# diku-kmc/kleenexlang

Hardware: AMD Instinct MI355X
Metric: input GB/s + % HBM-read roofline, apache_log.kex over 10 GiB synthetic log (higher is better)
Workload: dtype u8

## Files before the change

### kleenexlang_amd/csrc/engine/kx_dfkernels.inc

```

struct DfDev {
  const uint32_t* img; uint32_t words;
  uint32_t off_pool, deadh, esch, starth, K, C;
  const uint16_t* start_of_state;
  uint32_t orig_c4, hshift;
  uint32_t short_consts, debug;
  uint32_t nstates;
  uint32_t J;
  uint32_t wide;
  const uint4* sl_fmap;
  const uint32_t* sl_back; const uint8_t* sl_nleaves; const uint8_t* sl_fin_leaf; const uint8_t* sl_cls;
  const uint32_t* sl_pcoff; const uint8_t* sl_pcpool; const uint32_t* sl_pend; const uint32_t* sl_defoff; const uint32_t* sl_defpc; const uint16_t* sl_q;
  uint32_t sl_Lm, sl_npc, sl_on;
};
constexpr uint32_t DF_HOLE_MAX = 4096, DF_HOLE_FIRST = 1024, DF_SL_LEAVES = 32;
struct __attribute__((aligned(8))) DfRec { uint32_t x, y; };
constexpr uint32_t DFREC_OWN = 0x80000000u, DFREC_HOLE = 0x80000000u, DFREC_HOLE_FIRST = 0x40000000u;
constexpr uint32_t DF_MERGE_WINDOW_MAX = 64;
constexpr uint32_t DF_STEP_MAX = 126, DF_HOLE_LEN_MAX = 0xFFFFu, DF_HOLE_CNT_MAX = 0x3FFFu, DF_WBASE_PIECES = 32;
constexpr DfRec dfrec_pack(uint32_t start, uint32_t middle, uint32_t lenA, uint32_t len, uint32_t kA, uint32_t kB) {
  return DfRec{(start >> 3) | ((middle >> 3) << 13) | (kA << 26), len | (lenA << 13) | (kB << 25)};
}
constexpr DfRec dfrec_pack_hole(uint32_t side_first, uint32_t entries, bool first, uint32_t len) {
  return DfRec{side_first, len | (entries << 16) | (first ? DFREC_HOLE_FIRST : 0u) | DFREC_HOLE};
// ... 457 lines not shown
    for (uint32_t t = 0; t < plen; ++t) {
      if (t == HALF) { mid = h; lenA = len; kA = kc; }
      const uint2 e = L.ent(h + L.c8(in[pos + t]));
      const uint32_t nh = e.x & 0xFFFFu;
      if (nh == dead) { atomicMin(&flags->fail_pos, (unsigned long long)(pos + t)); return; }
      if (nh == esc) { flags->df_esc = 1; return; }
      h = nh; len += e.y >> 24; kc += (e.y >> 23) & 1u;
    }
    if (plen <= HALF) { mid = h; lenA = len; kA = kc; }
    if (kc > 0) atomicMax(&flags->emit_kmax, kc);
    if (((pos >> 6) & (DF_WBASE_PIECES - 1)) == 0) wbase[(pos >> 6) / DF_WBASE_PIECES] = cum;
    rec[pos >> 6] = dfrec_pack(h0, mid, lenA, len, kA, kc - kA);
    cum += len; pos += plen;
  }
  spill[m] = cum;
  if (head_len == n) flags->end_state = h;
}

__global__ void k_dlen(uint32_t nblk, const uint32_t* __restrict__ own, const uint32_t* __restrict__ spill, uint32_t* __restrict__ len,
                       unsigned long long* __restrict__ wsum) {
  __shared__ unsigned long long red[1024];
  const uint32_t m = blockIdx.x * blockDim.x + threadIdx.x;
  uint32_t mylen = 0;
  if (m < nblk) { mylen = own[m] + spill[m]; len[m] = mylen; }
  red[threadIdx.x] = mylen;
  __syncthreads();
  for (uint32_t s = blockDim.x >> 1; s > 0; s >>= 1) {
    if (threadIdx.x < s) red[threadIdx.x] += red[threadIdx.x + s];
    __syncthreads();
  }
  if (threadIdx.x == 0) wsum[blockIdx.x] = red[0];
}

template <bool GENERAL>
__global__ void k_dmap(const uint8_t* __restrict__ in, uint64_t n, uint32_t q_in, uint64_t cap, uint8_t* __restrict__ map_out,
                       uint32_t* __restrict__ status, DevTables T) {
  extern __shared__ __attribute__((aligned(16))) uint32_t smem[];
  Lds L = stage_tables<GENERAL>(T, smem);
  if (blockIdx.x || threadIdx.x) return;
  __shared__ uint8_t M[2][256];
  const uint32_t C = T.nclasses;
  uint32_t h = (OFF_FWD + q_in * C * 4) >> T.hshift, cur = 0;
  uint32_t nl = T.nleaves[q_in];
  for (uint32_t l = 0; l < nl; ++l) M[0][l] = (uint8_t)l;
  uint64_t pos = 0;
  bool constant = nl == 1, dead = false;
  while (pos < n && pos < cap && !constant && !dead) {
    const uint64_t a8 = pos & ~7ull;
    uint64_t x = 0;
    if (a8 + 8 <= n) { const uint2 v = *reinterpret_cast<const uint2*>(in + a8); x = (uint64_t)v.x | ((uint64_t)v.y << 32); }
    else for (uint64_t i = a8; i < n; ++i) x |= (uint64_t)in[i] << (8 * (i - a8));
    for (uint32_t b = (uint32_t)pos & 7u; b < 8u && pos < n && pos < cap && !constant; ++b, ++pos) {
      const uint32_t e = L.next(h, (uint32_t)(x >> (8 * b)) & 0xFFu);
      const uint32_t nh = e & 0xFFFFu;
      if (nh == T.deadh) { dead = true; break; }
      const uint32_t row = L.ra(e >> 16);
      const uint32_t nq = ((nh << T.hshift) - OFF_FWD) / (C * 4);
      const uint32_t nnl = T.nleaves[nq];
      constant = true;
      for (uint32_t l = 0; l < nnl; ++l) {
        const uint32_t p = (L.w(row + l * 4) >> 2) & 0xFFu;
        M[cur ^ 1][l] = M[cur][p < nl ? p : 0];
        constant = constant && M[cur ^ 1][l] == M[cur ^ 1][0];
      }
      cur ^= 1; h = nh; nl = nnl;
    }
// ... 26 lines not shown
  asm volatile("s_mov_b64 %[sv], exec\n"
               "v_cmpx_lt_u32_e32 vcc, 0, %[m]\n"
               "ds_write_b32 %[d], %[w0]\n"
               "v_cmpx_lt_u32_e32 vcc, 1, %[m]\n"
               "ds_write_b32 %[d], %[w1] offset:4\n"
               "v_cmpx_lt_u32_e32 vcc, 2, %[m]\n"
               "ds_write_b32 %[d], %[w2] offset:8\n"
               "v_cmpx_lt_u32_e32 vcc, 3, %[m]\n"
               "ds_write_b32 %[d], %[w3] offset:12\n"
               "s_mov_b64 exec, %[sv]\n"
               : [sv] "=&s"(sv) : [m] "v"(m), [d] "v"(d), [w0] "v"(w[0]), [w1] "v"(w[1]), [w2] "v"(w[2]), [w3] "v"(w[3]) : "vcc", "memory");
}

#ifndef KX_PRIO_CONSTANTS
#define KX_PRIO_CONSTANTS 2
#endif
#ifndef KX_PRIO_FLUSH
#define KX_PRIO_FLUSH 1
#endif
constexpr int HALF_BYTES = HALF;

template <int CONSTS>
__device__ __forceinline__ void df_step_gen(uint32_t& h, uint32_t byte_now, uint32_t byte_out, uint64_t& o, uint8_t* __restrict__ dst,
                                            const DfLds& L, const DfDev& D) {
  const uint2 e = L.ent(h + L.c8(byte_now));
  h = e.x & 0xFFFFu;
  const uint32_t cp = E_COPY(e.y), dl = e.y >> 24;
  if (cp) dst[o] = (uint8_t)byte_out;
  if (dl > cp) { const uint32_t src = D.off_pool + (E_AID(e.y) << 4); for (uint32_t i = 0; i < dl - cp; ++i) dst[o + cp + i] = L.base[src + i]; }
  o += dl;
}

template <int WAVES, int K, bool HALF = false>
__global__ __launch_bounds__(WAVES * 64) void k_demit(const uint8_t* __restrict__ in, uint64_t n, uint64_t blk, uint64_t blk_inv,
                                                      uint64_t npieces_total, const DfRec* __restrict__ rec, const uint32_t* __restrict__ wbase,
                                                      const uint32_t* __restrict__ spill, const unsigned long long* __restrict__ off,
                                                      Flags* __restrict__ flags, uint32_t stgb, uint32_t jbytes, uint32_t maxcnt,
                                                      uint8_t* __restrict__ out, const uint32_t* __restrict__ side, DfDev D) {
  extern __shared__ __attribute__((aligned(16))) uint32_t smem[];
  DfLds L = df_stage(D, smem);
  if ((uint32_t)(uintptr_t)smem != 0u) __builtin_trap();
  constexpr int NB = HALF ? HALF_BYTES : PIECE, NW = NB / 4;
  const uint32_t wave = threadIdx.x >> 6, lane = threadIdx.x & 63;
  const uint32_t stga = ((D.words + 3) & ~3u) * 4 + wave * (stgb + 16 + jbytes);
  uint8_t* stg = (uint8_t*)smem + stga;
  const uint32_t jarea = stga + stgb + 16;
  const uint64_t nunits = HALF ? npieces_total * 2 : npieces_total;
  const uint64_t nwi = (nunits + 63) / 64;
  const uint64_t oend_all = flags->total_len;
  const uint64_t one_piece_blocks = (uint64_t)__builtin_amdgcn_readfirstlane(blk == (uint64_t)PIECE ? 1 : 0);
  struct Operands { uint32_t w[NW]; uint32_t wp; uint2 r; uint32_t wb; uint64_t off0; uint32_t sp0; };
  auto request = [&](uint64_t it_, Operands& o) {
    if (it_ >= nwi) return;
    {
      const uint64_t itu = ((uint64_t)(uint32_t)__builtin_amdgcn_readfirstlane((int)(uint32_t)(it_ >> 32)) << 32) | (uint32_t)__builtin_amdgcn_readfirstlane((int)(uint32_t)it_);
      const uint64_t pf = itu * (HALF ? 32u : 64u);
      const uint64_t mf = __umul64hi(pf, blk_inv) + pf * one_piece_blocks;
      uint32_t vw, vm;
      asm("v_mov_b32 %0, %1" : "=v"(vw) : "s"((uint32_t)(pf / DF_WBASE_PIECES)));
      asm("v_mov_b32 %0, %1" : "=v"(vm) : "s"((uint32_t)mf));
      o.wb = wbase[vw]; o.off0 = off[vm]; o.sp0 = spill[vm];
    }
    const uint64_t u = it_ * 64 + lane;
    const bool ok = u < nunits;
    const uint64_t pc = HALF ? u >> 1 : u;
    const uint64_t ustart = ok ? (HALF ? pc * PIECE + (u & 1) * HALF_BYTES : pc * PIECE) : n;
    if constexpr (HALF) {
      if (ustart + HALF_BYTES <= n) {
        const uint4* p = reinterpret_cast<const uint4*>(in + ustart);
        const uint4 v0 = p[0], v1 = p[1];
        o.w[0] = v0.x; o.w[1] = v0.y; o.w[2] = v0.z; o.w[3] = v0.w; o.w[4] = v1.x; o.w[5] = v1.y; o.w[6] = v1.z; o.w[7] = v1.w;
      } else {
#pragma unroll
        for (int i = 0; i < NW; ++i) {
          uint32_t x = 0;
#pragma unroll
          for (int bb = 0; bb < 4; ++bb) { const uint64_t a = ustart + 4 * i + bb; if (a < n) x |= (uint32_t)in[a] << (8 * bb); }
          o.w[i] = x;
        }
      }
    } else load_piece(in, n, ustart, o.w);
    o.wp = *reinterpret_cast<const uint32_t*>(ok && ustart >= 4 ? in + ustart - 4 : reinterpret_cast<const uint8_t*>(D.img));
    o.r = *reinterpret_cast<const uint2*>(rec + (ok ? pc : 0));
  };
  Operands nx, cur;
  request((uint64_t)blockIdx.x * WAVES + wave, nx);
  cur = nx;
  unsigned long long tk[6] = {0, 0, 0, 0, 0, 0};
  auto stamp = [&]() -> unsigned long long {
    if (!(D.debug & 64u)) return 0ull;
    asm volatile("s_waitcnt vmcnt(0) lgkmcnt(0)" ::: "memory");
    return __builtin_amdgcn_s_memtime();
  };
  for (uint64_t it = (uint64_t)blockIdx.x * WAVES + wave; it < nwi; it += (uint64_t)gridDim.x * WAVES) {
    const unsigned long long t0 = stamp();
    const uint64_t unit = it * 64 + lane;
    const bool valid = unit < nunits;
    const uint64_t piece = HALF ? unit >> 1 : unit;
    const uint32_t half = HALF ? (uint32_t)unit & 1u : 0u;
    const uint64_t ustart = piece * PIECE + half * HALF_BYTES;
    const int plen = valid ? (int)(n <= ustart ? 0 : n - ustart < (uint64_t)NB ? n - ustart : NB) : 0;
    uint32_t w[NW];
#pragma unroll
    for (int i = 0; i < NW; ++i) w[i] = cur.w[i];
    const uint32_t wp = cur.wp;
    const DfRec rc{cur.r.x, cur.r.y};
    const bool hole = valid && dfrec_hole(rc);
    const uint32_t len = hole ? dfrec_hole_len(rc) : dfrec_len(rc), lenA = hole ? len : dfrec_lenA(rc);
    const uint32_t kA = HALF ? (half ? dfrec_kB(rc) : dfrec_kA(rc)) : dfrec_kA(rc), kB = HALF ? 0u : dfrec_kB(rc);
    const uint32_t hA = HALF ? (half ? dfrec_middle(rc) : dfrec_start(rc)) : dfrec_start(rc), hB = dfrec_middle(rc);
    const uint32_t ulen = valid ? (HALF ? (half ? len - lenA : lenA) : len) : 0u;
    const uint32_t before = wave_scan_incl(ulen) - ulen;
    const uint64_t obase = cur.off0 + (cur.wb & ~DFREC_OWN) + ((cur.wb & DFREC_OWN) ? cur.sp0 : 0u);
    const uint64_t ostart = valid ? obase + before : oend_all, oend = valid ? ostart + ulen : oend_all;
    const unsigned long long vmask = __ballot(valid);
    const uint32_t nvalid = (uint32_t)__popcll(vmask);
    uint32_t first = 0;
    bool taken = false;
    unsigned long long t2 = stamp();
    tk[0] += t2 - t0;
    if (hole && half == 0) {
      const uint32_t cntE = dfrec_hole_entries(rc), e0 = dfrec_hole_side(rc);
      uint64_t u = dfrec_hole_first(rc) ? piece * PIECE - K : piece * PIECE, o = ostart;
      for (uint32_t x = 0; x < cntE; ++x) {
        const uint32_t ee = side[e0 + x], pc = (ee >> 1) & 0x3FFFFFFFu;
        if (ee & 1u) out[o++] = in[u];
        if (pc < D.sl_npc) for (uint32_t b = D.sl_pcoff[pc]; b < D.sl_pcoff[pc + 1]; ++b) out[o++] = D.sl_pcpool[b];
        if (!(ee >> 31)) ++u;
      }
    }
    while (first < nvalid) {
      if (first == 0) request(it + (uint64_t)gridDim.x * WAVES, nx);
      const uint64_t gs = wave_read64(ostart, first);
      const uint64_t abase = gs & ~15ull;
      const bool fits = valid && lane >= first && (oend - abase) <= (uint64_t)stgb && plen == NB && !hole;
      const unsigned long long fm = __ballot(fits) >> first;
      uint32_t cnt = fm == ~0ull ? 64u - first : (uint32_t)__builtin_ctzll(~fm);
      if (cnt > maxcnt) cnt = maxcnt;
      if (cnt == 0) {
        if (lane == first && hole) {
        } else
        if (lane == first) {
          uint32_t h = hA;
          uint64_t o = ostart;
          for (int t = 0; t < plen; ++t) {
            const int ts = t - K;
            const uint32_t bn = (w[t >> 2] >> ((t & 3) * 8)) & 0xFFu;
            const uint32_t bo_ = ts >= 0 ? (w[ts >> 2] >> ((ts & 3) * 8)) & 0xFFu : (wp >> ((4 + ts) * 8)) & 0xFFu;
            df_step_gen<0>(h, bn, bo_, o, out, L, D);
          }
        }
        first += 1;
        continue;
      }
      const uint32_t lastl = first + cnt - 1;
      const bool active = lane >= first && lane <= lastl;
      const uint32_t o0 = stga + (uint32_t)(ostart - abase);
      const bool inplace = jbytes == 0;
      const uint32_t need = active ? (kA + kB) * 4u : 0u;
      const uint32_t incl = wave_scan_incl(need);
      const uint32_t jtotal = (uint32_t)__builtin_amdgcn_readlane((int)incl, 63);
      const bool jfit = !inplace && jtotal <= jbytes;
      const unsigned long long t3 = stamp();
      tk[2] += t3 - t2;
      if (active && jfit) {
        uint32_t oA = o0, pA = jarea + incl - need;
        if constexpr (HALF) {
          if (D.wide) { if constexpr (K == 1) piece_dfwalk1cw_k1(w, wp, hA, oA, pA); else piece_dfwalk1cw_k2(w, wp, hA, oA, pA); }
          else { if constexpr (K == 1) piece_dfwalk1c_k1(w, wp, hA, oA, pA); else piece_dfwalk1c_k2(w, wp, hA, oA, pA); }
        } else {
          uint32_t oB = o0 + lenA, pB = pA + 4u * kA;
          if (D.wide) {
            if constexpr (K == 1) piece_dfwalk2cw_k1(w, wp, hA, oA, hB, oB, pA, pB);
            else piece_dfwalk2cw_k2(w, wp, hA, oA, hB, oB, pA, pB);
          } else {
            if constexpr (K == 1) piece_dfwalk2c_k1(w, wp, hA, oA, hB, oB, pA, pB);
            else piece_dfwalk2c_k2(w, wp, hA, oA, hB, oB, pA, pB);
          }
        }
      }
      uint32_t njobs = jfit ? jtotal >> 2 : 0u;
      if (!jfit) {
        if (!inplace && lane == first) atomicAdd(&flags->emit_ovf, cnt);
        if (active) {
          for (int ch = 0; ch < (HALF ? 1 : 2); ++ch) {
            uint32_t h = ch ? hB : hA;
            uint64_t o = (uint64_t)(o0 - stga) + (ch ? lenA : 0u);
            for (int t = ch * HALF_BYTES; t < (ch + 1) * HALF_BYTES; ++t) {
              const int ts = t - K;
              const uint32_t bn = (w[t >> 2] >> ((t & 3) * 8)) & 0xFFu;
// ... 9 lines not shown
      __builtin_amdgcn_s_setprio(KX_PRIO_CONSTANTS);
      for (uint32_t j0 = 0; j0 < njobs; j0 += 64) {
        const uint32_t j = j0 + lane;
        uint32_t l = 0, d = 0, off0 = 0;
        if (j < njobs) {
          const uint32_t jw = *reinterpret_cast<const uint32_t*>((const uint8_t*)smem + jarea + 4 * j);
          const uint32_t e = *reinterpret_cast<const uint32_t*>(L.base + (jw & 0xFFFFu) + 4);
          const uint32_t cp = E_COPY(e);
          l = (e >> 24) - cp;
          d = stga + (((jw >> 16) - stga) & 0xFFFFu) + cp;
          off0 = D.off_pool + (E_AID(e) << 4);
        }
        const uint32_t tob = (0u - d) & 3u, nh = l < tob ? l : tob, rem = l - nh;
        const uint32_t src = off0 + nh * ((l + 15u) & ~15u), d1 = d + nh;
        const uint32_t v0 = *reinterpret_cast<const uint32_t*>(L.base + off0);
        uint4 wv = *reinterpret_cast<const uint4*>(L.base + src);
        put_bytes3(nh, d, v0);
        for (uint32_t base = 0;; base += 16) {
          const uint32_t left = rem > base ? rem - base : 0u, m = left >> 2 < 4u ? left >> 2 : 4u;
          const uint32_t w4[4] = {wv.x, wv.y, wv.z, wv.w};
          put_dwords4(m, d1 + base, w4);
          const uint32_t nt = left < 16u ? left & 3u : 0u;
          const uint32_t tw = m == 0 ? wv.x : m == 1 ? wv.y : m == 2 ? wv.z : wv.w;
          put_bytes3(nt, d1 + base + 4u * m, tw);
          if (!__any(rem > base + 16u)) break;
          wv = *reinterpret_cast<const uint4*>(L.base + src + base + 16u);
        }
      }
      wave_lds_fence();
      __builtin_amdgcn_s_setprio(KX_PRIO_FLUSH);
      const unsigned long long t5 = stamp();
      tk[4] += t5 - t4;
      if (lastl + 1 >= nvalid) { cur = nx; taken = true; }
      const uint64_t ge = wave_read64(oend, lastl);
      const uint64_t fs = (gs + 15) & ~15ull, fe = ge & ~15ull;
      if (fs >= fe) {
        for (uint64_t x = gs + lane; x < ge; x += 64) out[x] = stg[x - abase];
      } else {
        if (gs + lane < fs) out[gs + lane] = stg[gs + lane - abase];
        if (fe + lane < ge) out[fe + lane] = stg[fe + lane - abase];
        for (uint64_t x = fs + (uint64_t)lane * 16; x < fe; x += 1024)
          *reinterpret_cast<uint4*>(out + x) = *reinterpret_cast<const uint4*>(stg + (x - abase));
      }
      wave_lds_fence();
      __builtin_amdgcn_s_setprio(0);
      t2 = stamp();
      tk[5] += t2 - t5;
      first = lastl + 1;
    }
    if (!taken) cur = nx;
  }
  if ((D.debug & 64u) && lane == 0)
    for (int i = 0; i < 6; ++i) atomicAdd(&flags->dbg[i], tk[i]);
}
```

### kleenexlang_amd/csrc/engine/kx_engine.hip

```cpp
#include <hip/hip_runtime.h>
#include <fcntl.h>
#include <sys/stat.h>
#include <unistd.h>

#include <cerrno>
#include <condition_variable>
#include <cstdint>
#include <algorithm>
#include <deque>
#include <mutex>
#include <chrono>
#include <thread>
#include <cstdio>
#include <cstdlib>
#include <cstring>
#include <string>
#include <type_traits>
#include <vector>

#include "../../../include/kxhip.h"
#include "../../../include/kxp_format.h"
#include "kx_delayed.h"

namespace {
// ... 1798 lines not shown
    *out_len = olen;
    return 0;
  }
};

struct kx_program {
  std::vector<Stage> stages;
  void* actbuf[2][2] = {{nullptr, nullptr}, {nullptr, nullptr}};
  size_t actcap[2][2] = {{0, 0}, {0, 0}};
  kx_config cfg = [] { kx_config c{}; c.block_threads = 512; return c; }();
  std::vector<Arena*> arenas;
  void* stagebuf[2] = {nullptr, nullptr};
  size_t stagecap[2] = {0, 0};
  hipEvent_t ev[KX_NKERNELS + 1] = {};
  bool have_events = false;
  int ncu = 256;
  std::vector<ActionRunner*> act_runners;
  BatchWs* batch = nullptr;
  FieldWs* fields = nullptr;
  FieldListWs* field_list = nullptr;
};

struct kx_shard {
  kx_program* prog; Stage* st; uint32_t stage; Arena* arena = nullptr;
  const DevTables* T = nullptr;
  const uint8_t* in; uint64_t n; int is_first, is_last; hipStream_t stream;
  uint64_t seg; uint32_t nseg, nblk, Lc, ngroups;
  uint64_t* seg_pos; uint16_t* seg_state; uint16_t* chk; Flags* flags;
  uint8_t *bs_start, *bs_merged, *bs_mstart, *E, *d_map; uint32_t *bs_len, *len, *d_const, *ctot;
  PieceRec* prec; uint16_t* merge_piece;
  unsigned long long *off, *wsum, *woff;
  Flags hflags{}; uint64_t head_len = 0; bool have_end = false; uint64_t out_len = 0; uint32_t init_shift = 0, init_leaf = 0;
  uint32_t df_qin = 0;
  bool df = false; DfRec* dfrec = nullptr; uint32_t *df_wbase = nullptr, *df_own = nullptr, *df_spill = nullptr, *side = nullptr; uint32_t side_cap = 0; std::vector<uint8_t> df_tail; uint64_t df_body = 0;
  uint32_t endId() const {
    if (!df) return st->stateOf(hflags.end_state);
    const uint32_t i = st->df.indexOf(hflags.end_state);
    return i < st->df.states.size() ? st->df.states[i].q : st->q0;
  }
  kx_stats stats{};
};

namespace {

size_t pad4(size_t x) { return (x + 3) & ~(size_t)3; }

thread_local int g_force_jl = -1;

int parseStage(const uint8_t*& c, const uint8_t* end, Stage& S, const kx_config& cfg, bool dry = false) {
  if (end < c || (size_t)(end - c) < 64) return setErr(KX_E_BLOB, "truncated stage header");
  uint32_t h[16];
  memcpy(h, c, 64); c += 64;
  if (h[0] != KXP_STAGE_MAGIC) return setErr(KX_E_BLOB, "bad stage magic");
  const uint32_t nstates = h[1], C = h[2], q0 = h[3], nactions = h[5], nops = h[6], nconsts = h[7], cpl = h[8];
  const uint32_t Lm = h[9], nback = h[10], npc = h[11], pcpl = h[12], nsync = h[13];
  const size_t sc = (size_t)nstates * C;
  {
    const unsigned long long need = 256ull + pad4(sc * 2) + sc * 4 + (unsigned long long)nstates * 4 + ((unsigned long long)nactions + 1) * 4 +
                                    (unsigned long long)nops * 8 + ((unsigned long long)nconsts + 1) * 4 + pad4(cpl) + sc * 4 + 2 * pad4(nstates) +
                                    (unsigned long long)nback * Lm * 4 + ((unsigned long long)npc + 1) * 4 + pad4(pcpl) + (unsigned long long)Lm * 4 +
                                    (unsigned long long)nsync * C * 4 + (unsigned long long)nsync * 4;
    if (nstates > 0xFFFFu || C > 256 || Lm > 256 || need > (unsigned long long)(end - c)) return setErr(KX_E_BLOB, "truncated stage body");
  }
  const uint8_t* cls = c; c += 256;
  const uint16_t* delta = (const uint16_t*)c; c += pad4(sc * 2);
  c += sc * 4;
  c += (size_t)nstates * 4;
// ... 637 lines not shown

uint32_t kx_num_stages(const kx_program* p) { return p ? (uint32_t)p->stages.size() : 0; }
int kx_stage_has_actions(const kx_program* p, uint32_t stage) { return p && stage < p->stages.size() && p->stages[stage].act ? 1 : 0; }

static int shardBegin(kx_program* p, uint32_t stage, const void* d_in, size_t n, int is_first, int is_last,
                      void* stream, kx_shard** out, bool internal) {
  if (!p || !out || stage >= p->stages.size()) return setErr(KX_E_ARG, "bad program/stage");
  if (!internal && p->stages[stage].act) return setErr(KX_E_ARG, "a stage with register actions cannot be sharded (kx_stage_has_actions)");
  if (n && (!d_in || ((uintptr_t)d_in & 15))) return setErr(KX_E_ARG, "input must be 16-byte aligned");
  if ((uint64_t)n >> 38) return setErr(KX_E_ARG, "a shard holds at most 256 GiB (piece indices are 32-bit); stream larger inputs in windows");
  auto* s = new kx_shard;
  s->prog = p; s->st = &p->stages[stage]; s->stage = stage;
  s->T = s->st->has_alt && s->st->use_alt ? &s->st->Talt : &s->st->T;
  s->in = (const uint8_t*)d_in; s->n = n; s->is_first = is_first; s->is_last = is_last; s->stream = (hipStream_t)stream;
  s->seg = p->cfg.segment_bytes;
  if (s->seg == 0) {
    const uint64_t slots = (uint64_t)p->ncu * 1024;
    const uint64_t m = (n + slots * 65536 - 1) / (slots * 65536) ? (n + slots * 65536 - 1) / (slots * 65536) : 1;
    s->seg = ((n + m * slots - 1) / (m * slots) + 511) & ~(uint64_t)511;
    if (s->seg < 4096) s->seg = 4096;
  }
  uint64_t ns = n ? (n + s->seg - 1) / s->seg : 1;
  if (ns > 0x7FFFFFF0ull) { delete s; return setErr(KX_E_ARG, "input too large for the configured segment size"); }
  s->nseg = (uint32_t)ns; s->nblk = s->nseg; s->Lc = s->st->maxleaves;
  const uint32_t bt = p->cfg.block_threads;
  s->ngroups = (s->nblk + bt - 1) / bt;
  if (p->arenas.empty()) p->arenas.push_back(new Arena);
  s->arena = p->arenas.back(); p->arenas.pop_back();
  Arena& A = *s->arena;
  s->df = s->st->has_df && n > 0;
  if (s->df && s->st->df_given_up) s->df = false;
  if (s->df && s->st->df_skip) { s->df = false; --s->st->df_skip; }
  s->side_cap = s->df && s->st->D.sl_on ? (uint32_t)(n / 8 < (1u << 22) ? (n / 8 > (1u << 18) ? n / 8 : (1u << 18)) : (1u << 22)) : 0u;
  size_t need = 4096 + (s->df ? (n / PIECE + 16) * sizeof(DfRec) + (n / PIECE / DF_WBASE_PIECES + 8) * 4 + 256 + (size_t)s->nseg * 8 + 512 + (size_t)s->side_cap * 4 + 256 : 0) + (size_t)s->nseg * (8 + 2) + (n / HALF + 32) * 2 + sizeof(Flags) +
                (size_t)s->nblk * ((size_t)s->Lc * 5 + 3 + 4 + 8 + 2 + 4) + (size_t)s->ngroups * 16 + KX_MAX_LEAVES + 64 +
                (n / PIECE + 16) * 8 + 256 * 32;
  int rc = A.reserve(need);
  if (rc) { p->arenas.push_back(s->arena); delete s; return rc; }
  A.reset();
  s->seg_pos = A.take<uint64_t>(s->nseg); s->seg_state = A.take<uint16_t>(s->nseg);
  s->chk = A.take<uint16_t>(n / HALF + 32); s->flags = A.take<Flags>(1);
  s->bs_start = A.take<uint8_t>((size_t)s->nblk * s->Lc); s->bs_len = A.take<uint32_t>((size_t)s->nblk * s->Lc);
  s->bs_merged = A.take<uint8_t>(s->nblk); s->bs_mstart = A.take<uint8_t>(s->nblk); s->E = A.take<uint8_t>(s->nblk);
  s->len = A.take<uint32_t>(s->nblk); s->off = A.take<unsigned long long>(s->nblk);
  s->wsum = A.take<unsigned long long>(s->ngroups); s->woff = A.take<unsigned long long>(s->ngroups);
  s->d_map = A.take<uint8_t>(KX_MAX_LEAVES); s->d_const = A.take<uint32_t>(4);
  s->prec = A.take<PieceRec>(n / PIECE + 16);
  s->merge_piece = A.take<uint16_t>(s->nblk); s->ctot = A.take<uint32_t>(s->nblk);
  if (s->df) { s->dfrec = A.take<DfRec>(n / PIECE + 16); s->df_wbase = A.take<uint32_t>(n / PIECE / DF_WBASE_PIECES + 8); s->df_own = A.take<uint32_t>(s->nblk); s->df_spill = A.take<uint32_t>(s->nblk); s->side = s->side_cap ? A.take<uint32_t>(s->side_cap) : nullptr; }
  if (!p->have_events) {
    for (auto& e : p->ev) if (hipEventCreate(&e) != hipSuccess) { p->arenas.push_back(s->arena); delete s; return setErr(KX_E_HIP, "hipEventCreate failed"); }
    p->have_events = true;
  }
  s->stats.in_bytes = n;
  *out = s;
  return 0;
}

int kx_shard_begin(kx_program* p, uint32_t stage, const void* d_in, size_t n, int is_first, int is_last,
                   void* stream, kx_shard** out) {
  return shardBegin(p, stage, d_in, n, is_first, is_last, stream, out, false);
}

static int readFlags(kx_shard* s) {
  HIPCHECK(hipMemcpyAsync(&s->hflags, s->flags, sizeof(Flags), hipMemcpyDeviceToHost, s->stream));
  HIPCHECK(hipStreamSynchronize(s->stream));
  return 0;
}

static void fillFwd(kx_shard* s, kx_fwd_summary* out) {
  out->synced = s->have_end ? 1 : 0;
  out->end_state = s->have_end ? s->endId() : 0;
  out->head_len = s->head_len;
  out->fail_pos = s->hflags.fail_pos;
}

static int generalForward(kx_shard* s) {
  kx_program* p = s->prog; Stage& S = *s->st;
  const uint32_t bt = p->cfg.block_threads;
  const bool timing = p->cfg.collect_timing;
  const uint32_t grid = (s->nseg + bt - 1) / bt;
  if (timing) HIPCHECK(hipEventRecord(p->ev[1], s->stream));
// ... 224 lines not shown
#undef KX_LAUNCH_BACKLEN
  if (timing) HIPCHECK(hipEventRecord(p->ev[1], s->stream));
  HIPCHECK(hipGetLastError());
  if (!s->is_first) {
    hipLaunchKernelGGL(k_shard_map, dim3(1), dim3(64), 0, s->stream, s->nblk, nle, s->bs_start, s->bs_merged,
                       s->bs_mstart, s->Lc, s->d_map, s->d_const);
    HIPCHECK(hipMemcpyAsync(out->start_leaf, s->d_map, nle, hipMemcpyDeviceToHost, s->stream));
    HIPCHECK(hipMemcpyAsync(&out->constant, s->d_const, 4, hipMemcpyDeviceToHost, s->stream));
  }
  HIPCHECK(hipStreamSynchronize(s->stream));
  if (timing) s->stats.kernel_ms[KX_K_BACKLEN] = evMs(p->ev[0], p->ev[1]);
  return 0;
}

int kx_shard_resolve(kx_shard* s, uint32_t end_leaf, uint64_t* out_len) {
  if (!s || !out_len) return setErr(KX_E_ARG, "null argument");
  kx_program* p = s->prog; Stage& S = *s->st;
  if (s->is_last) end_leaf = S.h_fin_leaf[s->endId()];
  if (end_leaf >= S.h_nleaves[s->endId()]) return setErr(KX_E_ARG, "end leaf out of range");
  if (s->n == 0) {
    s->init_shift = s->is_first ? S.h_init_len[end_leaf] : 0;
    s->out_len = s->init_shift;
    *out_len = s->out_len;
    s->init_leaf = end_leaf;
    return 0;
  }
  const uint32_t bt = p->cfg.block_threads;
  const bool timing = p->cfg.collect_timing;
  if (s->df) {
    if (timing) HIPCHECK(hipEventRecord(p->ev[0], s->stream));
    hipLaunchKernelGGL(k_dlen, dim3(s->ngroups), dim3(bt), 0, s->stream, s->nblk, s->df_own, s->df_spill, s->len, s->wsum);
    hipLaunchKernelGGL(k_scan_groups, dim3(1), dim3(1024), 0, s->stream, s->ngroups, s->wsum, s->woff, s->flags);
    hipLaunchKernelGGL(k_scan_blocks, dim3(s->ngroups), dim3(bt), 0, s->stream, s->nblk, s->len, s->woff, s->off);
    if (timing) HIPCHECK(hipEventRecord(p->ev[1], s->stream));
    HIPCHECK(hipGetLastError());
    const uint32_t K = S.df.K;
    uint8_t lastb[kxdf::DF_MAX_K] = {0, 0, 0, 0};
    const uint32_t nb = s->n < K ? (uint32_t)s->n : K;
    HIPCHECK(hipMemcpyAsync(lastb + (K - nb), s->in + (s->n - nb), nb, hipMemcpyDeviceToHost, s->stream));
    int rc = readFlags(s);
    if (rc) return rc;
    if (timing) s->stats.kernel_ms[KX_K_RESOLVE] = evMs(p->ev[0], p->ev[1]);
    if (S.df.indexOf(s->hflags.end_state) >= S.df.states.size()) return setErr(KX_E_ARG, "internal: the shard did not end in a state of the delayed form");
    const kxdf::DfState& E = S.df.states[S.df.indexOf(s->hflags.end_state)];
    s->df_tail.clear();
    for (const auto& d : E.def)
      if (d.first < S.df_pc_len.size()) s->df_tail.insert(s->df_tail.end(), S.h_pool.begin() + S.df_pc_off[d.first], S.h_pool.begin() + S.df_pc_off[d.first] + S.df_pc_len[d.first]);
    for (uint32_t j = 0; j < K; ++j) {
      const kxdf::Slot& g = E.pend[j];
      const kxdf::Kind kd = g.size() == 1 ? g[0] : g[end_leaf < g.size() ? end_leaf : 0];
      if (kd & 1u) s->df_tail.push_back(lastb[j]);
      const uint32_t pc = kd >> 1;
      if (pc < S.df_pc_len.size()) s->df_tail.insert(s->df_tail.end(), S.h_pool.begin() + S.df_pc_off[pc], S.h_pool.begin() + S.df_pc_off[pc] + S.df_pc_len[pc]);
    }
    s->init_shift = 0; s->init_leaf = 0;
    s->df_body = s->hflags.total_len;
    s->out_len = s->df_body + s->df_tail.size();
    *out_len = s->out_len;
    return 0;
  }
  if (timing) HIPCHECK(hipEventRecord(p->ev[0], s->stream));
  hipLaunchKernelGGL(k_resolve_leaf, dim3(s->ngroups), dim3(bt), 0, s->stream, s->nblk, end_leaf, s->bs_start, s->bs_merged, s->bs_mstart, s->Lc, s->E);
  hipLaunchKernelGGL(k_resolve, dim3(s->ngroups), dim3(bt), 0, s->stream, s->nblk, s->E, s->bs_len, s->Lc, s->len, s->wsum);
  hipLaunchKernelGGL(k_scan_groups, dim3(1), dim3(1024), 0, s->stream, s->ngroups, s->wsum, s->woff, s->flags);
  hipLaunchKernelGGL(k_scan_blocks, dim3(s->ngroups), dim3(bt), 0, s->stream, s->nblk, s->len, s->woff, s->off);
  if (S.general)
// ... 36 lines not shown
    return 0;
  }
  const bool timing = p->cfg.collect_timing;
  const uint64_t npieces = (s->n + PIECE - 1) / PIECE;
  const uint64_t nwi = (npieces + 63) / 64;
  if (s->df) {
    const size_t lds_cap = 160 * 1024, tab = ((size_t)S.D.words * 4 + 15) & ~(size_t)15;
    int W = 12;
    { const int v = (int)p->cfg.emit_waves; if (v == 4 || v == 8 || v == 12 || v == 16) W = v; }
    const size_t per_wave = ((lds_cap - tab) / W) & ~(size_t)63;
    const double olen = 64.0 * (double)s->out_len / (double)s->n;
    const uint32_t kmax = s->hflags.emit_kmax < 64 ? s->hflags.emit_kmax : 64;
    double kper = s->hflags.emit_kn ? 1.1 * (double)s->hflags.emit_ksum / (double)s->hflags.emit_kn + 1.0 : (double)kmax + 1;
    if (kper > kmax + 1) kper = kmax + 1;
    size_t stgb = 0, jbytes = 0; uint32_t maxcnt = 64;
    auto plan = [&](double ol, double kp) {
      for (uint32_t R = 1; R <= 64; ++R) {
        const uint32_t c = (64 + R - 1) / R;
        size_t st = (((size_t)(c * ol * 1.05) + 64) + 63) & ~(size_t)63, jb = ((size_t)(c * kp + 16) * 4 + 63) & ~(size_t)63;
        if (st < 1024) st = 1024;
        if (st + 16 + jb <= per_wave || c == 1) { maxcnt = c; jbytes = jb; stgb = per_wave - 16 - jb; break; }
      }
    };
    plan(olen, kper);
    bool halfmode = maxcnt <= 32 && (W == 12 || W == 16);
    if (p->cfg.emit_half) halfmode = p->cfg.emit_half == 2 && (W == 12 || W == 16);
    if (halfmode) plan(olen / 2, kper / 2 + 0.5);
    if (stgb > 49152) stgb = 49152;
    stgb &= ~(size_t)15;
    const uint64_t nwi_df = halfmode ? (npieces * 2 + 63) / 64 : nwi;
    const uint64_t wantg = (nwi_df + W - 1) / W;
    const uint32_t grid = (uint32_t)(wantg < (uint64_t)p->ncu ? wantg : (uint64_t)p->ncu);
    const size_t elds = tab + (size_t)W * (stgb + 16 + jbytes);
    const uint64_t ppb = s->seg / PIECE, blk_inv = ppb > 1 ? ~0ull / ppb + 1 : 0;
    if (timing) HIPCHECK(hipEventRecord(p->ev[0], s->stream));
#define KX_LAUNCH_DEMIT(WV, KK)                                                                                                    \
  hipLaunchKernelGGL((k_demit<WV, KK>), dim3(grid), dim3(WV * 64), elds, s->stream, s->in, s->n, s->seg, blk_inv, npieces, s->dfrec, s->df_wbase, \
                     s->df_spill, s->off, s->flags, (uint32_t)stgb, (uint32_t)jbytes, maxcnt, (uint8_t*)d_out, s->side, S.D)
#define KX_LAUNCH_DEMIT_K(WV) do { if (S.df.K == 1) KX_LAUNCH_DEMIT(WV, 1); else KX_LAUNCH_DEMIT(WV, 2); } while (0)
#define KX_LAUNCH_DEMIT_H(WV, KK)                                                                                                    \
  hipLaunchKernelGGL((k_demit<WV, KK, true>), dim3(grid), dim3(WV * 64), elds, s->stream, s->in, s->n, s->seg, blk_inv, npieces, s->dfrec, s->df_wbase, \
                     s->df_spill, s->off, s->flags, (uint32_t)stgb, (uint32_t)jbytes, maxcnt, (uint8_t*)d_out, s->side, S.D)
    if (halfmode) {
      if (W == 16) { if (S.df.K == 1) KX_LAUNCH_DEMIT_H(16, 1); else KX_LAUNCH_DEMIT_H(16, 2); }
      else { if (S.df.K == 1) KX_LAUNCH_DEMIT_H(12, 1); else KX_LAUNCH_DEMIT_H(12, 2); }
    } else
    if (W == 16) KX_LAUNCH_DEMIT_K(16); else if (W == 12) KX_LAUNCH_DEMIT_K(12); else if (W == 8) KX_LAUNCH_DEMIT_K(8); else KX_LAUNCH_DEMIT_K(4);
#undef KX_LAUNCH_DEMIT_H
#undef KX_LAUNCH_DEMIT_K
#undef KX_LAUNCH_DEMIT
    if (timing) HIPCHECK(hipEventRecord(p->ev[1], s->stream));
    HIPCHECK(hipGetLastError());
    if (!s->df_tail.empty())
      HIPCHECK(hipMemcpyAsync((uint8_t*)d_out + s->df_body, s->df_tail.data(), s->df_tail.size(), hipMemcpyHostToDevice, s->stream));
    uint32_t ovf = 0;
    const bool debug = getenv("KX_DEBUG") != nullptr;
    if (timing || debug) HIPCHECK(hipMemcpyAsync(&ovf, &s->flags->emit_ovf, 4, hipMemcpyDeviceToHost, s->stream));
    HIPCHECK(hipStreamSynchronize(s->stream));
    if (timing) s->stats.kernel_ms[KX_K_EMIT] = evMs(p->ev[0], p->ev[1]);
    s->stats.emit_overflow_pieces = ovf;
    S.df_streak = 0;
    if (debug && (S.D.debug & 64u)) {
      Flags hf; HIPCHECK(hipMemcpy(&hf, s->flags, sizeof(Flags), hipMemcpyDeviceToHost));
      double tot = 0; for (int i = 0; i < 6; ++i) tot += (double)hf.dbg[i];
      fprintf(stderr, "[kx] emit timeline, delayed form (share of wave time): operands+logic %.3f round-logic %.3f walk %.3f constants %.3f flush %.3f; ticks/wave-iteration %.0f\n",
              hf.dbg[0] / tot, hf.dbg[2] / tot, hf.dbg[3] / tot, hf.dbg[4] / tot, hf.dbg[5] / tot, tot / (double)nwi);
    }
    if (debug) fprintf(stderr, "[kx] emit (delayed form, K=%u, %u product states, image %zu B)%s: W=%d stg=%zu jobs=%zu maxcnt=%u kmax=%u kavg=%.2f olen=%.1f overflow=%u of %llu pieces\n",
                       S.df.K, S.df.nP, (size_t)S.D.words * 4, halfmode ? ", a lane = half a piece" : "", W, stgb, jbytes, maxcnt, kmax, s->hflags.emit_kn ? (double)s->hflags.emit_ksum / s->hflags.emit_kn : -1.0, olen, ovf, (unsigned long long)npieces);
    return 0;
  }
  const size_t lds_cap = 160 * 1024, tab = (S.lds_bytes + 15) & ~(size_t)15;
  int W = tab + 12 * (size_t)EMIT_WAVE_LDS_MIN <= lds_cap ? 12 : tab + 8 * (size_t)EMIT_WAVE_LDS_MIN <= lds_cap ? 8 : 4;
  { const int v = (int)p->cfg.emit_waves; if ((v == 4 || v == 8 || v == 12) && v <= W) W = v; }
  const size_t per_wave = ((lds_cap - tab) / W) & ~(size_t)255;
// ... 542 lines not shown
```

Before: 1122.

## Precompute per-group output bases in a small kernel and use 32-bit wave offsets

A new kernel k_dobase computes each 32-piece group's 64-bit output base from wbase, spill and off before the emit launch. The emit kernel then does one 64-bit load per wave instead of three dependent loads and the block-index multiply. Per-lane offsets become 32-bit scans and readlanes relative to that uniform base, replacing 64-bit wave reads. The cost is an extra small kernel launch and buffer. The offsets also now assume a wave's output span fits in 32 bits.

Result: no change. 1112 (-0.9%).

```diff
diff --git a/kleenexlang_amd/csrc/engine/kx_dfkernels.inc b/kleenexlang_amd/csrc/engine/kx_dfkernels.inc
--- a/kleenexlang_amd/csrc/engine/kx_dfkernels.inc
+++ b/kleenexlang_amd/csrc/engine/kx_dfkernels.inc
@@ -513,6 +513,15 @@
   if (threadIdx.x == 0) wsum[blockIdx.x] = red[0];
 }
 
+__global__ void k_dobase(uint64_t nbase, uint64_t blk_inv, const uint32_t* __restrict__ wbase, const uint32_t* __restrict__ spill,
+                         const unsigned long long* __restrict__ off, unsigned long long* __restrict__ obase) {
+  const uint64_t i = (uint64_t)blockIdx.x * blockDim.x + threadIdx.x;
+  if (i >= nbase) return;
+  const uint64_t pf = i * DF_WBASE_PIECES, m = blk_inv ? __umul64hi(pf, blk_inv) : pf;
+  const uint32_t wb = wbase[i];
+  obase[i] = off[m] + (wb & ~DFREC_OWN) + ((wb & DFREC_OWN) ? spill[m] : 0u);
+}
+
 template <bool GENERAL>
 __global__ void k_dmap(const uint8_t* __restrict__ in, uint64_t n, uint32_t q_in, uint64_t cap, uint8_t* __restrict__ map_out,
                        uint32_t* __restrict__ status, DevTables T) {
@@ -605,9 +614,8 @@
 }
 
 template <int WAVES, int K, bool HALF = false>
-__global__ __launch_bounds__(WAVES * 64) void k_demit(const uint8_t* __restrict__ in, uint64_t n, uint64_t blk, uint64_t blk_inv,
-                                                      uint64_t npieces_total, const DfRec* __restrict__ rec, const uint32_t* __restrict__ wbase,
-                                                      const uint32_t* __restrict__ spill, const unsigned long long* __restrict__ off,
+__global__ __launch_bounds__(WAVES * 64) void k_demit(const uint8_t* __restrict__ in, uint64_t n, uint64_t npieces_total,
+                                                      const DfRec* __restrict__ rec, const unsigned long long* __restrict__ obase_of,
                                                       Flags* __restrict__ flags, uint32_t stgb, uint32_t jbytes, uint32_t maxcnt,
                                                       uint8_t* __restrict__ out, const uint32_t* __restrict__ side, DfDev D) {
   extern __shared__ __attribute__((aligned(16))) uint32_t smem[];
@@ -620,19 +628,15 @@
   const uint32_t jarea = stga + stgb + 16;
   const uint64_t nunits = HALF ? npieces_total * 2 : npieces_total;
   const uint64_t nwi = (nunits + 63) / 64;
-  const uint64_t oend_all = flags->total_len;
-  const uint64_t one_piece_blocks = (uint64_t)__builtin_amdgcn_readfirstlane(blk == (uint64_t)PIECE ? 1 : 0);
-  struct Operands { uint32_t w[NW]; uint32_t wp; uint2 r; uint32_t wb; uint64_t off0; uint32_t sp0; };
+  struct Operands { uint32_t w[NW]; uint32_t wp; uint2 r; uint64_t ob; };
   auto request = [&](uint64_t it_, Operands& o) {
     if (it_ >= nwi) return;
     {
       const uint64_t itu = ((uint64_t)(uint32_t)__builtin_amdgcn_readfirstlane((int)(uint32_t)(it_ >> 32)) << 32) | (uint32_t)__builtin_amdgcn_readfirstlane((int)(uint32_t)it_);
       const uint64_t pf = itu * (HALF ? 32u : 64u);
-      const uint64_t mf = __umul64hi(pf, blk_inv) + pf * one_piece_blocks;
-      uint32_t vw, vm;
+      uint32_t vw;
       asm("v_mov_b32 %0, %1" : "=v"(vw) : "s"((uint32_t)(pf / DF_WBASE_PIECES)));
-      asm("v_mov_b32 %0, %1" : "=v"(vm) : "s"((uint32_t)mf));
-      o.wb = wbase[vw]; o.off0 = off[vm]; o.sp0 = spill[vm];
+      o.ob = obase_of[vw];
     }
     const uint64_t u = it_ * 64 + lane;
     const bool ok = u < nunits;
@@ -683,9 +687,8 @@
     const uint32_t kA = HALF ? (half ? dfrec_kB(rc) : dfrec_kA(rc)) : dfrec_kA(rc), kB = HALF ? 0u : dfrec_kB(rc);
     const uint32_t hA = HALF ? (half ? dfrec_middle(rc) : dfrec_start(rc)) : dfrec_start(rc), hB = dfrec_middle(rc);
     const uint32_t ulen = valid ? (HALF ? (half ? len - lenA : lenA) : len) : 0u;
-    const uint32_t before = wave_scan_incl(ulen) - ulen;
-    const uint64_t obase = cur.off0 + (cur.wb & ~DFREC_OWN) + ((cur.wb & DFREC_OWN) ? cur.sp0 : 0u);
-    const uint64_t ostart = valid ? obase + before : oend_all, oend = valid ? ostart + ulen : oend_all;
+    const uint32_t oend32 = wave_scan_incl(ulen), ostart32 = oend32 - ulen;
+    const uint64_t obase = ((uint64_t)(uint32_t)__builtin_amdgcn_readfirstlane((int)(uint32_t)(cur.ob >> 32)) << 32) | (uint32_t)__builtin_amdgcn_readfirstlane((int)(uint32_t)cur.ob);
     const unsigned long long vmask = __ballot(valid);
     const uint32_t nvalid = (uint32_t)__popcll(vmask);
     uint32_t first = 0;
@@ -694,7 +697,7 @@
     tk[0] += t2 - t0;
     if (hole && half == 0) {
       const uint32_t cntE = dfrec_hole_entries(rc), e0 = dfrec_hole_side(rc);
-      uint64_t u = dfrec_hole_first(rc) ? piece * PIECE - K : piece * PIECE, o = ostart;
+      uint64_t u = dfrec_hole_first(rc) ? piece * PIECE - K : piece * PIECE, o = obase + ostart32;
       for (uint32_t x = 0; x < cntE; ++x) {
         const uint32_t ee = side[e0 + x], pc = (ee >> 1) & 0x3FFFFFFFu;
         if (ee & 1u) out[o++] = in[u];
@@ -704,9 +707,11 @@
     }
     while (first < nvalid) {
       if (first == 0) request(it + (uint64_t)gridDim.x * WAVES, nx);
-      const uint64_t gs = wave_read64(ostart, first);
+      const uint32_t gs32 = (uint32_t)__builtin_amdgcn_readlane((int)ostart32, (int)first);
+      const uint64_t gs = obase + gs32;
       const uint64_t abase = gs & ~15ull;
-      const bool fits = valid && lane >= first && (oend - abase) <= (uint64_t)stgb && plen == NB && !hole;
+      const uint32_t skew = (uint32_t)gs & 15u;
+      const bool fits = valid && lane >= first && (oend32 - gs32) + skew <= stgb && plen == NB && !hole;
       const unsigned long long fm = __ballot(fits) >> first;
       uint32_t cnt = fm == ~0ull ? 64u - first : (uint32_t)__builtin_ctzll(~fm);
       if (cnt > maxcnt) cnt = maxcnt;
@@ -715,7 +720,7 @@
         } else
         if (lane == first) {
           uint32_t h = hA;
-          uint64_t o = ostart;
+          uint64_t o = obase + ostart32;
           for (int t = 0; t < plen; ++t) {
             const int ts = t - K;
             const uint32_t bn = (w[t >> 2] >> ((t & 3) * 8)) & 0xFFu;
@@ -728,7 +733,7 @@
       }
       const uint32_t lastl = first + cnt - 1;
       const bool active = lane >= first && lane <= lastl;
-      const uint32_t o0 = stga + (uint32_t)(ostart - abase);
+      const uint32_t o0 = stga + (ostart32 - gs32) + skew;
       const bool inplace = jbytes == 0;
       const uint32_t need = active ? (kA + kB) * 4u : 0u;
       const uint32_t incl = wave_scan_incl(need);
@@ -804,7 +809,7 @@
       const unsigned long long t5 = stamp();
       tk[4] += t5 - t4;
       if (lastl + 1 >= nvalid) { cur = nx; taken = true; }
-      const uint64_t ge = wave_read64(oend, lastl);
+      const uint64_t ge = obase + (uint32_t)__builtin_amdgcn_readlane((int)oend32, (int)lastl);
       const uint64_t fs = (gs + 15) & ~15ull, fe = ge & ~15ull;
       if (fs >= fe) {
         for (uint64_t x = gs + lane; x < ge; x += 64) out[x] = stg[x - abase];
diff --git a/kleenexlang_amd/csrc/engine/kx_engine.hip b/kleenexlang_amd/csrc/engine/kx_engine.hip
--- a/kleenexlang_amd/csrc/engine/kx_engine.hip
+++ b/kleenexlang_amd/csrc/engine/kx_engine.hip
@@ -1854,7 +1854,7 @@
   unsigned long long *off, *wsum, *woff;
   Flags hflags{}; uint64_t head_len = 0; bool have_end = false; uint64_t out_len = 0; uint32_t init_shift = 0, init_leaf = 0;
   uint32_t df_qin = 0;
-  bool df = false; DfRec* dfrec = nullptr; uint32_t *df_wbase = nullptr, *df_own = nullptr, *df_spill = nullptr, *side = nullptr; uint32_t side_cap = 0; std::vector<uint8_t> df_tail; uint64_t df_body = 0;
+  bool df = false; DfRec* dfrec = nullptr; uint32_t *df_wbase = nullptr, *df_own = nullptr, *df_spill = nullptr, *side = nullptr; unsigned long long* df_obase = nullptr; uint32_t side_cap = 0; std::vector<uint8_t> df_tail; uint64_t df_body = 0;
   uint32_t endId() const {
     if (!df) return st->stateOf(hflags.end_state);
     const uint32_t i = st->df.indexOf(hflags.end_state);
@@ -2558,7 +2558,7 @@
   if (s->df && s->st->df_given_up) s->df = false;
   if (s->df && s->st->df_skip) { s->df = false; --s->st->df_skip; }
   s->side_cap = s->df && s->st->D.sl_on ? (uint32_t)(n / 8 < (1u << 22) ? (n / 8 > (1u << 18) ? n / 8 : (1u << 18)) : (1u << 22)) : 0u;
-  size_t need = 4096 + (s->df ? (n / PIECE + 16) * sizeof(DfRec) + (n / PIECE / DF_WBASE_PIECES + 8) * 4 + 256 + (size_t)s->nseg * 8 + 512 + (size_t)s->side_cap * 4 + 256 : 0) + (size_t)s->nseg * (8 + 2) + (n / HALF + 32) * 2 + sizeof(Flags) +
+  size_t need = 4096 + (s->df ? (n / PIECE + 16) * sizeof(DfRec) + (n / PIECE / DF_WBASE_PIECES + 8) * (4 + 8) + 512 + (size_t)s->nseg * 8 + 512 + (size_t)s->side_cap * 4 + 256 : 0) + (size_t)s->nseg * (8 + 2) + (n / HALF + 32) * 2 + sizeof(Flags) +
                 (size_t)s->nblk * ((size_t)s->Lc * 5 + 3 + 4 + 8 + 2 + 4) + (size_t)s->ngroups * 16 + KX_MAX_LEAVES + 64 +
                 (n / PIECE + 16) * 8 + 256 * 32;
   int rc = A.reserve(need);
@@ -2573,7 +2573,7 @@
   s->d_map = A.take<uint8_t>(KX_MAX_LEAVES); s->d_const = A.take<uint32_t>(4);
   s->prec = A.take<PieceRec>(n / PIECE + 16);
   s->merge_piece = A.take<uint16_t>(s->nblk); s->ctot = A.take<uint32_t>(s->nblk);
-  if (s->df) { s->dfrec = A.take<DfRec>(n / PIECE + 16); s->df_wbase = A.take<uint32_t>(n / PIECE / DF_WBASE_PIECES + 8); s->df_own = A.take<uint32_t>(s->nblk); s->df_spill = A.take<uint32_t>(s->nblk); s->side = s->side_cap ? A.take<uint32_t>(s->side_cap) : nullptr; }
+  if (s->df) { s->dfrec = A.take<DfRec>(n / PIECE + 16); s->df_wbase = A.take<uint32_t>(n / PIECE / DF_WBASE_PIECES + 8); s->df_obase = A.take<unsigned long long>(n / PIECE / DF_WBASE_PIECES + 8); s->df_own = A.take<uint32_t>(s->nblk); s->df_spill = A.take<uint32_t>(s->nblk); s->side = s->side_cap ? A.take<uint32_t>(s->side_cap) : nullptr; }
   if (!p->have_events) {
     for (auto& e : p->ev) if (hipEventCreate(&e) != hipSuccess) { p->arenas.push_back(s->arena); delete s; return setErr(KX_E_HIP, "hipEventCreate failed"); }
     p->have_events = true;
@@ -2864,6 +2864,11 @@
     hipLaunchKernelGGL(k_dlen, dim3(s->ngroups), dim3(bt), 0, s->stream, s->nblk, s->df_own, s->df_spill, s->len, s->wsum);
     hipLaunchKernelGGL(k_scan_groups, dim3(1), dim3(1024), 0, s->stream, s->ngroups, s->wsum, s->woff, s->flags);
     hipLaunchKernelGGL(k_scan_blocks, dim3(s->ngroups), dim3(bt), 0, s->stream, s->nblk, s->len, s->woff, s->off);
+    {
+      const uint64_t nbase = ((s->n + PIECE - 1) / PIECE + DF_WBASE_PIECES - 1) / DF_WBASE_PIECES;
+      const uint64_t ppb = s->seg / PIECE, blk_inv = ppb > 1 ? ~0ull / ppb + 1 : 0;
+      hipLaunchKernelGGL(k_dobase, dim3((uint32_t)((nbase + bt - 1) / bt)), dim3(bt), 0, s->stream, nbase, blk_inv, s->df_wbase, s->df_spill, s->off, s->df_obase);
+    }
     if (timing) HIPCHECK(hipEventRecord(p->ev[1], s->stream));
     HIPCHECK(hipGetLastError());
     const uint32_t K = S.df.K;
@@ -2966,15 +2971,14 @@
     const uint64_t wantg = (nwi_df + W - 1) / W;
     const uint32_t grid = (uint32_t)(wantg < (uint64_t)p->ncu ? wantg : (uint64_t)p->ncu);
     const size_t elds = tab + (size_t)W * (stgb + 16 + jbytes);
-    const uint64_t ppb = s->seg / PIECE, blk_inv = ppb > 1 ? ~0ull / ppb + 1 : 0;
     if (timing) HIPCHECK(hipEventRecord(p->ev[0], s->stream));
 #define KX_LAUNCH_DEMIT(WV, KK)                                                                                                    \
-  hipLaunchKernelGGL((k_demit<WV, KK>), dim3(grid), dim3(WV * 64), elds, s->stream, s->in, s->n, s->seg, blk_inv, npieces, s->dfrec, s->df_wbase, \
-                     s->df_spill, s->off, s->flags, (uint32_t)stgb, (uint32_t)jbytes, maxcnt, (uint8_t*)d_out, s->side, S.D)
+  hipLaunchKernelGGL((k_demit<WV, KK>), dim3(grid), dim3(WV * 64), elds, s->stream, s->in, s->n, npieces, s->dfrec, s->df_obase, \
+                     s->flags, (uint32_t)stgb, (uint32_t)jbytes, maxcnt, (uint8_t*)d_out, s->side, S.D)
 #define KX_LAUNCH_DEMIT_K(WV) do { if (S.df.K == 1) KX_LAUNCH_DEMIT(WV, 1); else KX_LAUNCH_DEMIT(WV, 2); } while (0)
 #define KX_LAUNCH_DEMIT_H(WV, KK)                                                                                                    \
-  hipLaunchKernelGGL((k_demit<WV, KK, true>), dim3(grid), dim3(WV * 64), elds, s->stream, s->in, s->n, s->seg, blk_inv, npieces, s->dfrec, s->df_wbase, \
-                     s->df_spill, s->off, s->flags, (uint32_t)stgb, (uint32_t)jbytes, maxcnt, (uint8_t*)d_out, s->side, S.D)
+  hipLaunchKernelGGL((k_demit<WV, KK, true>), dim3(grid), dim3(WV * 64), elds, s->stream, s->in, s->n, npieces, s->dfrec, s->df_obase, \
+                     s->flags, (uint32_t)stgb, (uint32_t)jbytes, maxcnt, (uint8_t*)d_out, s->side, S.D)
     if (halfmode) {
       if (W == 16) { if (S.df.K == 1) KX_LAUNCH_DEMIT_H(16, 1); else KX_LAUNCH_DEMIT_H(16, 2); }
       else { if (S.df.K == 1) KX_LAUNCH_DEMIT_H(12, 1); else KX_LAUNCH_DEMIT_H(12, 2); }
```
